# kento/TEZip

Measured on AMD Instinct MI355X. Metric: frames/sec (predict+delta-encode), 512x512 seq, higher is better.
Workload: dtype f32; 1 GPU; 512x512x3 synthetic turbulence stack, 80 frames per GPU (ONE 80-frame sequence), SWP 20-frame windows, warm_up 0, lossy rel 1e-3, entropy remap on; PredNet (3,48,96,192) glorot seed 123

## Files before the change

### tezip_amd/build.py

```python
import os
import subprocess
import sys
from concurrent.futures import ThreadPoolExecutor

HERE = os.path.dirname(os.path.abspath(__file__))
CSRC = os.path.join(HERE, "csrc")
SOURCES = ["tz_api.hip", "tz_codec.hip", "tz_prednet.hip"]
HEADERS = ["tz_internal.h", "tz_math.hip.h", "tz_conv_kernels.hip.h", "tz_wino_kernels.hip.h", "tz_wino_geometry.inc.h", "tz_wino_transform.inc.h",
           "tz_wino_output.inc.h", "tz_wino_epilogue.inc.h", os.path.join("..", "..", "include", "tezip_hip.h")]
LIB = os.path.join(CSRC, "libtezip_hip.so")
HIPCC = os.environ.get("HIPCC", "/opt/rocm/bin/hipcc")
FLAGS = (["-D" + d for d in os.environ.get("TEZIP_DEFINES", "").split()] if os.environ.get("TEZIP_DEFINES") else []) + ["--offload-arch=gfx950", "-O3", "-std=c++17", "-fPIC", "-ffp-contract=off",
         "-fhip-fp32-correctly-rounded-divide-sqrt", "-fno-fast-math", "-Wall", "-Wno-unused-function"]


STAMP = os.path.join(CSRC, ".build_flags")


def _flags_changed():
    try:
        return open(STAMP).read() != " ".join(FLAGS)
    except OSError:
        return True


def _stale(target, deps):
    if not os.path.exists(target):
        return True
    t = os.path.getmtime(target)
    return any(os.path.getmtime(d) > t for d in deps)


def build(force=False, verbose=False):
    hdrs = [os.path.join(CSRC, h) for h in HEADERS]
    force = force or _flags_changed()
    objs, jobs = [], []
    for s in SOURCES:
        src = os.path.join(CSRC, s)
        obj = os.path.join(CSRC, s.replace(".hip", ".o"))
        objs.append(obj)
        if force or _stale(obj, [src] + hdrs):
            jobs.append([HIPCC] + FLAGS + ["-c", src, "-o", obj])

    def run(cmd):
        if verbose:
            print(" ".join(cmd), flush=True)
        r = subprocess.run(cmd, capture_output=True, text=True)
        if r.returncode != 0:
            raise RuntimeError("hipcc failed:\n%s\n%s" % (" ".join(cmd), r.stderr[-8000:]))
        return r.stderr

    if jobs:
        with ThreadPoolExecutor(max_workers=len(jobs)) as ex:
            for err in ex.map(run, jobs):
                if verbose and err.strip():
                    print(err)
    if jobs or force or _stale(LIB, objs):
        run([HIPCC, "--offload-arch=gfx950", "-shared", "-fPIC", "-pthread", "-o", LIB] + objs)
        with open(STAMP, "w") as f:
            f.write(" ".join(FLAGS))
    return LIB


if __name__ == "__main__":
    print(build(force="--force" in sys.argv, verbose=True))
```

### tezip_amd/csrc/tz_prednet.hip

```cpp
#include <algorithm>
#include <atomic>
#include <cmath>

#include "tz_conv_kernels.hip.h"
#include "tz_wino_kernels.hip.h"

struct Seg {
    int row_off, C;
    int up;
    int half = 0;
    int row(int c) const { return half && c >= half ? 4 + c - half : c; }
};
struct PackedConv {
    float* d_W = nullptr;
    float* d_Wimg = nullptr;
    float* d_Wblk = nullptr;
    float* d_Wblk0 = nullptr;
    bool pos_finite = false;
    std::vector<float> h_W0;
    float* d_Wlat = nullptr;
    float* d_Wwino = nullptr;
    float* d_Wwino2 = nullptr;
    const float* d_zero = nullptr;
    float* d_bias = nullptr;
    int nslots = 0, ncols = 0, NT = 1, ncb = 1;
    int wino_finite = 0;
    bool wino_all_finite = false;
    std::vector<Seg> segs;
};

enum { UNI_G0 = 0, UNI_C0 = 1, UNI_AHAT0 = 2 };
enum { UNI_USE_WINO_INIT = 1, UNI_USE_WINO_CELL = 2, UNI_USE_TILES = 4, UNI_USE_ALL = 7 };

struct tz_model {
    int L = 0;
    int stack[TZ_MAX_LEVELS] = {0}, rstack[TZ_MAX_LEVELS] = {0};
    std::vector<std::vector<float>> w;
    int Hp = 0, Wp = 0, maxB = 0;
    int cap = 0;
    bool prepared = false;
    float *R0[TZ_MAX_LEVELS] = {0}, *C0[TZ_MAX_LEVELS] = {0}, *Ahat0[TZ_MAX_LEVELS] = {0}, *G0[TZ_MAX_LEVELS] = {0};
    float *G0f[TZ_MAX_LEVELS] = {0}, *C0f[TZ_MAX_LEVELS] = {0};
    int ring[3][TZ_MAX_LEVELS] = {{0}};
    int tring[3][TZ_MAX_LEVELS] = {{0}};
    const float* uni[3][TZ_MAX_LEVELS] = {{0}};
    int uniform_mask = 0;
    int dead[TZ_MAX_LEVELS] = {0}, dead_gate[TZ_MAX_LEVELS] = {0}, dead_a[TZ_MAX_LEVELS] = {0};
    bool dead0 = false;
    bool dead0_hold = false;
    bool deadf[TZ_MAX_LEVELS] = {false};
    bool deadhalf[TZ_MAX_LEVELS] = {false};
    bool e0_dirty = false;
    float *E[TZ_MAX_LEVELS] = {0}, *R1[TZ_MAX_LEVELS] = {0};
    float* P[TZ_MAX_LEVELS] = {0};
    int Pcap[TZ_MAX_LEVELS] = {0};
    std::vector<signed char> epart_choice;
    PackedConv a_conv[TZ_MAX_LEVELS], gate_t1[TZ_MAX_LEVELS], ahat0_t1;
    PackedConv gate_nf[TZ_MAX_LEVELS];
    float* d_zero = nullptr;
    int e0s = 0;
    int* d_idx = nullptr;
    std::vector<void*> allocs;
    const float* a_k(int l) const { return w[2 * l].data(); }
    const float* a_b(int l) const { return w[2 * l + 1].data(); }
    const float* ahat_k(int l) const { return w[2 * (L - 1) + 2 * l].data(); }
    const float* ahat_b(int l) const { return w[2 * (L - 1) + 2 * l + 1].data(); }
    int gate_base(int g) const {
        static const int pos[4] = {2, 1, 0, 3};
        return 2 * (L - 1) + 2 * L + pos[g] * 2 * L;
    }
    const float* g_k(int g, int l) const { return w[gate_base(g) + 2 * l].data(); }
    const float* g_b(int g, int l) const { return w[gate_base(g) + 2 * l + 1].data(); }
    int gate_cin(int l) const { return rstack[l] + 2 * stack[l] + (l < L - 1 ? rstack[l + 1] : 0); }
};

static int dmalloc(tz_ctx* ctx, tz_model* m, void** p, size_t bytes) {
    if (bytes == 0) bytes = 16;
    hipError_t e = hipMalloc(p, bytes);
    if (e != hipSuccess) return tz_fail(ctx, TZ_ERR_NOMEM, "hipMalloc(%zu) failed: %s", bytes, hipGetErrorString(e));
    m->allocs.push_back(*p);
    return tz_poison(ctx, *p, bytes);
}

struct ColSrc {
    const float* kernel;
    const float* bias;
    int Cin, Cout, ch;
};

static int collapse_set(int a, int d, int out[2]) {
    if (a == 0) {
        if (d == 0) { out[0] = 0; return 1; }
        out[0] = 1; out[1] = 2; return 2;
    }
    if (d == 0) { out[0] = 0; out[1] = 1; return 2; }
    out[0] = 2; return 1;
}

static int pack_conv(tz_ctx* ctx, tz_model* m, const std::vector<Seg>& segs, const std::vector<ColSrc>& cols, int NT,
                     PackedConv* pc) {
    int ncols = (int)cols.size();
    int nslots = 0;
    for (auto& s : segs) nslots += (s.up ? 16 : 9) * ((s.C + 15) / 16);
    std::vector<float> W((size_t)std::max(nslots, 1) * 16 * ncols, 0.0f), B(ncols, 0.0f);
    int slot = 0;
    bool pos_finite = true;
    auto put = [&](const Seg& s, int c0, const int* kys, int nky, const int* kxs, int nkx) {
        for (int kc = 0; kc < 16 && c0 + kc < s.C; ++kc)
            for (int col = 0; col < ncols; ++col) {
                const ColSrc& cs = cols[col];
                if (cs.ch < 0) continue;
                float v = 0.0f;
                bool first = true;
                for (int iy = 0; iy < nky; ++iy)
                    for (int ix = 0; ix < nkx; ++ix) {
                        float w = cs.kernel[((size_t)(kys[iy] * 3 + kxs[ix]) * cs.Cin + s.row_off + c0 + kc) * cs.Cout + cs.ch];
                        v = first ? w : v + w;
                        first = false;
                    }
                W[((size_t)slot * 16 + s.row(c0 + kc) - c0) * ncols + col] = v;
                if (s.half && c0 + kc < s.half && !std::isfinite(v)) pos_finite = false;
            }
        ++slot;
    };
    for (auto& s : segs)
        for (int c0 = 0; c0 < s.C; c0 += 16) {
            if (!s.up) {
                for (int tap = 0; tap < 9; ++tap) {
                    int ky = tap / 3, kx = tap % 3;
                    put(s, c0, &ky, 1, &kx, 1);
                }
            } else {
                for (int tp = 0; tp < 4; ++tp)
                    for (int cls = 0; cls < 4; ++cls) {
                        int kys[2], kxs[2];
// ... 302 lines not shown
    if (epi == EPI_POOL_ERR && !ups) return NT == 4 ? launch_wino_t<4, EPI_POOL_ERR, false>(ctx, a, nbatch) : launch_wino_t<3, EPI_POOL_ERR, false>(ctx, a, nbatch);
    return tz_fail(ctx, TZ_ERR_UNSUPPORTED, "no TZ-PA2 kernel for NT=%d epilogue=%d upsampled=%d", NT, epi, (int)ups);
}

static constexpr long long TZ_PA2_MIN_PIXELS = 256 * 256;
static constexpr size_t kPBytes = (size_t)160 << 20;
static constexpr double kEpartMinIdle = 0.06;
static constexpr int kEpartSteps = 3;
static constexpr int kEpartSamples = 4;
static constexpr float kEpartMinGain = 0.98f;
static int effective_contract(const tz_ctx* ctx) {
    if (ctx->contract) return ctx->contract;
    const tz_model* m = ctx->model;
    return m && (long long)m->Hp * m->Wp >= TZ_PA2_MIN_PIXELS ? 2 : 1;
}

#ifdef TZW_STAMPS
extern "C" int tz_debug_wino_stamps(unsigned long long* out) {
    return hipMemcpyFromSymbol(out, HIP_SYMBOL(tzw_stamps), sizeof(unsigned long long) * 8 * 4096 * 16) == hipSuccess ? 0 : -3;
}
#endif
extern "C" int tz_set_contract(tz_ctx* ctx, int contract) {
    if (!ctx) return TZ_ERR_INVALID;
    if (contract < 0 || contract > 2)
        return tz_fail(ctx, TZ_ERR_INVALID, "tz_set_contract: %d is not 0 (by frame size), 1 (TZ-PA1) or 2 (TZ-PA2)", contract);
    ctx->contract = contract;
    return TZ_OK;
}
extern "C" int tz_get_contract(tz_ctx* ctx) { return ctx ? effective_contract(ctx) : TZ_ERR_INVALID; }

extern "C" int tz_set_conv_impl(tz_ctx* ctx, int lds_dma) {
    if (!ctx) return TZ_ERR_INVALID;
    if (lds_dma < 0 || lds_dma > 5 || (lds_dma >> 1) > 2)
        return tz_fail(ctx, TZ_ERR_INVALID, "tz_set_conv_impl: %d is not 0 / 1 (+ 2 = never k_convlat, + 4 = k_convlat wherever eligible)", lds_dma);
    ctx->conv_impl = (lds_dma & 1) ? 1 : 0;
    const int lat = lds_dma >> 1;
    ctx->lat_mode = lat == 1 ? 0 : (lat == 2 ? 2 : 1);
    return TZ_OK;
}

struct LatPlan {
    bool use, wide;
    int blocks;
};
static LatPlan lat_plan(const tz_ctx* ctx, int NT, int epi, bool ups, bool fullk, const ConvArgs& a, int nbatch) {
    LatPlan lp = {false, false, 0};
    if (!(a.Wlat && a.nsrc > 0 && fullk && ctx->conv_impl && ctx->lat_mode && (NT == 3 || NT == 4) &&
          (epi == EPI_POOL_ERR || (epi == EPI_LSTM && NT == 4))))
        return lp;
    const int ts_ = (epi != EPI_POOL_ERR && ups) ? 8 : 4;
    const long long wg16 = (long long)a.ncb * a.tiles_x * a.tiles_y * nbatch;
    const long long rows_ = (a.H + ts_ - 1) / ts_ * (ts_ == 8 ? 4 : 1);
    const long long wglat1 = (long long)a.ncb * ((a.W + ts_ - 1) / ts_) * rows_ * nbatch;
    const long long wglat2 = (long long)a.ncb * ((a.W + 2 * ts_ - 1) / (2 * ts_)) * rows_ * nbatch;
    static const long long wide_min = getenv("TEZIP_LAT_WIDE_MIN") ? atoll(getenv("TEZIP_LAT_WIDE_MIN")) : 2560;
    lp.wide = wglat1 > wide_min;
    int slots = 0;
    for (int s = 0; s < a.nsrc; ++s) slots += a.src[s].cpt * (a.src[s].up ? 4 : 9);
    const double t16 = slots * 1.08 * (double)((wg16 + 255) / 256);
    const double per_slot = lp.wide ? 0.134 * (double)((wglat2 + 255) / 256) : std::max(0.105, 0.078 * (double)((wglat1 + 255) / 256));
    const double tlat = slots * per_slot * (ts_ == 8 ? 1.1 : 1.0) + 2.5;
    lp.use = wg16 <= 768 && (ctx->lat_mode == 2 || tlat < 0.9 * t16);
    lp.blocks = (int)(lp.wide ? wglat2 : wglat1);
    return lp;
}

static int launch_conv(tz_ctx* ctx, int NT, int epi, const ConvArgs& a, int nbatch, int wino_dead = 0, const float* wino3 = nullptr,
                       const float* wino3q = nullptr) {
    tz_prof_scope ps(ctx, TZP_CONV);
    bool ups = false, fullk = true;
    for (int s = 0; s < a.nsrc; ++s) {
        ups = ups || a.src[s].up;
        fullk = fullk && (a.src[s].C % 16) == 0;
        const long long hs = a.src[s].up ? a.H >> 1 : a.H, ws = a.src[s].up ? a.W >> 1 : a.W;
        fullk = fullk && hs * ws * a.src[s].pstride * 4 < (1LL << 32);
    }
    ps.sub = TZP_CONV_GEN;
    if (epi == EPI_RELU && a.nsrc == 1 && !ups && a.src[0].C == 3 && a.Cout == 3 && ctx->conv_impl) {
        ps.sub = TZP_CONV_SMALL;
        hipLaunchKernelGGL((k_conv_small<3, 3>), dim3(a.tiles_x * a.tiles_y * nbatch), dim3(256), 0, ctx->stream, a);
        TZ_HIP(ctx, hipGetLastError());
        return TZ_OK;
    }
    if (a.Wblk && a.nsrc > 0 && !a.src[0].up && a.src[0].pstride == 8 && ctx->conv_impl) {
        const int blocks = a.ncb * a.tiles_x * a.tiles_y * nbatch;
#define TZ_CASE16B(nt, e, u)                                                                                    \
    if (NT == nt && epi == e && ups == u) {                                                                     \
        ps.sub = TZP_CONV16B;                                                                                   \
        if (a.Wblk0) hipLaunchKernelGGL((k_conv16b<nt, e, u, true>), dim3(blocks), dim3(NTHR), 0, ctx->stream, a); \
        else hipLaunchKernelGGL((k_conv16b<nt, e, u>), dim3(blocks), dim3(NTHR), 0, ctx->stream, a);            \
        TZ_HIP(ctx, hipGetLastError());                                                                         \
        return TZ_OK;                                                                                           \
    }
        TZ_CASE16B(1, EPI_LSTM_PACKED, true) TZ_CASE16B(1, EPI_LSTM_PACKED, false)
        TZ_CASE16B(1, EPI_POOL_ERR, false) TZ_CASE16B(3, EPI_POOL_ERR, false) TZ_CASE16B(4, EPI_POOL_ERR, false)
#undef TZ_CASE16B
    }
    if (a.Wwino && effective_contract(ctx) == 2 && fullk && (epi == EPI_LSTM || epi == EPI_POOL_ERR || epi == EPI_RAW)) {
        ps.sub = TZP_WINO;
        return launch_wino(ctx, NT, epi, ups, a, nbatch, false, wino_dead, wino3, wino3q);
    }
    {
        const LatPlan lp = lat_plan(ctx, NT, epi, ups, fullk, a, nbatch);
        if (!lp.use) goto no_lat;
        const bool wide = lp.wide;
        const int blocks = lp.blocks;
        ps.sub = TZP_CONVLAT;
#define TZ_LAT(e, u)                                                                                          \
    do {                                                                                                      \
        if (wide) hipLaunchKernelGGL((k_convlat<e, u, 2>), dim3(blocks), dim3(256), 0, ctx->stream, a);       \
        else hipLaunchKernelGGL((k_convlat<e, u, 1>), dim3(blocks), dim3(256), 0, ctx->stream, a);            \
    } while (0)
        if (epi == EPI_LSTM && ups) TZ_LAT(EPI_LSTM, true);
        else if (epi == EPI_LSTM) TZ_LAT(EPI_LSTM, false);
        else TZ_LAT(EPI_POOL_ERR, false);
#undef TZ_LAT
        TZ_HIP(ctx, hipGetLastError());
        return TZ_OK;
    }
no_lat:
    if (a.Wimg && a.nsrc > 0 && fullk && ctx->conv_impl) {
#define TZ_CASE16(nt, e, u)                          \
    if (NT == nt && epi == e && ups == u) {          \
        ps.sub = TZP_CONV16;                         \
        launch_conv16_t<nt, e, u>(ctx, a, nbatch);   \
        TZ_HIP(ctx, hipGetLastError());              \
        return TZ_OK;                                \
    }
        TZ_CASE16(4, EPI_LSTM, false) TZ_CASE16(4, EPI_LSTM, true)
        TZ_CASE16(3, EPI_POOL_ERR, false) TZ_CASE16(4, EPI_POOL_ERR, false)
#undef TZ_CASE16
    }
#define TZ_CASE(nt, e, u)                                                   \
    if (NT == nt && epi == e && ups == u) {                                 \
        if (fullk) launch_conv_t<nt, e, u, true>(ctx, a, nbatch);           \
        else launch_conv_t<nt, e, u, false>(ctx, a, nbatch);                \
        TZ_HIP(ctx, hipGetLastError());                                     \
        return TZ_OK;                                                       \
    }
    TZ_CASE(1, EPI_RAW, false) TZ_CASE(4, EPI_RAW, false)
    TZ_CASE(1, EPI_RELU, false) TZ_CASE(3, EPI_RELU, false) TZ_CASE(4, EPI_RELU, false)
    TZ_CASE(4, EPI_LSTM, false) TZ_CASE(4, EPI_LSTM, true)
    TZ_CASE(1, EPI_LSTM_PACKED, false) TZ_CASE(1, EPI_LSTM_PACKED, true)
    TZ_CASE(1, EPI_POOL_ERR, false) TZ_CASE(3, EPI_POOL_ERR, false) TZ_CASE(4, EPI_POOL_ERR, false)
#undef TZ_CASE
    return tz_fail(ctx, TZ_ERR_UNSUPPORTED, "no conv kernel for NT=%d epilogue=%d upsampled=%d", NT, epi, (int)ups);
}

static void fill_srcs(ConvArgs& a, const PackedConv& pc, const float* const* ptrs, const long long* nstrides,
                      int pstride0 = 0) {
    a.nsrc = (int)pc.segs.size();
    for (int s = 0; s < a.nsrc; ++s) {
        a.src[s].p = ptrs[s];
        a.src[s].nstride = nstrides[s];
        a.src[s].C = pc.segs[s].half ? 8 : pc.segs[s].C;
        a.src[s].pstride = s == 0 && pstride0 ? pstride0 : pc.segs[s].C;
        a.src[s].up = pc.segs[s].up;
        a.src[s].cpt = (pc.segs[s].C + 15) / 16;
    }
    a.Wp = pc.d_W;
    a.Wimg = pc.d_Wimg;
    a.Wblk = pc.d_Wblk;
    a.Wblk0 = pc.d_Wblk0;
    a.Wlat = pc.d_Wlat;
    a.Wwino = pc.d_Wwino;
    a.zero = pc.d_zero;
// ... 164 lines not shown
        static const char* const names[2] = {"gates", "A"};
        for (int k = 0; k < 2; ++k) {
            if (!pcs[k] || !pcs[k]->d_Wwino) continue;
            *out[k] = pcs[k]->wino_finite >= d ? d : 0;
            if (log)
                fprintf(stderr, "[tezip] dead source, level %d %s: %d of %d leading positive-half blocks dead, %d skipped: %d of %d same-resolution stages%s\n",
                        l, names[k], d, m->stack[l] / 16, *out[k], 4 * *out[k], 2 * m->stack[l] / 4,
                        !on ? " (TEZIP_DEADSRC=0)" : (*out[k] < d ? " (a weight of those stages is not finite)" : ""));
        }
    }
    for (int l = 0; l < L; ++l) {
        const bool whole = l == 0 ? half0 : (m->stack[l] % 16 == 0 && m->stack[l] / 16 <= 64);
        const unsigned long long blocks = l == 0 ? 1ull : (m->stack[l] / 16 >= 64 ? ~0ull : (1ull << (m->stack[l] / 16)) - 1);
        m->deadhalf[l] = onh && whole && !(h_live[l] & blocks);
        if (logh)
            fprintf(stderr, "[tezip] dead half, level %d: Ahat0 +-0 over the whole plane: %s%s\n", l, m->deadhalf[l] ? "yes" : "no",
                    m->deadhalf[l] ? " (its writers store the live half alone)" : !onh ? " (TEZIP_DEADHALF=0)" : "");
    }
    if (half0 && (on0 || log0)) {
        const bool zero = !(h_live[0] & 1);
        m->dead0 = zero;
        PackedConv* pcs[2] = {L > 1 ? &m->a_conv[0] : nullptr, &m->gate_t1[0]};
        static const char* const names[2] = {"A", "gates"};
        for (int k = 0; k < 2; ++k) {
            if (!pcs[k]) continue;
            const bool form = pcs[k]->d_Wblk && !pcs[k]->h_W0.empty() && (k == 0 || pcs[k]->NT == 1), finite = pcs[k]->pos_finite;
            if (on0 && zero && form && finite) TZ_TRY(pack_block0_dead(ctx, m, pcs[k]));
            if (log0)
                fprintf(stderr, "[tezip] dead level 0, %s: positive half of E_0 +0 everywhere: %s, its k-step left out: %s%s\n", names[k],
                        zero ? "yes" : "no", pcs[k]->d_Wblk0 ? "yes" : "no",
                        pcs[k]->d_Wblk0 ? " (9 of 18 k-steps in block 0 of k_conv16b)"
                        : !zero         ? ""
                        : !on0          ? " (TEZIP_DEAD0=0)"
                        : !form         ? " (no k_conv16b form)"
                                        : " (a weight of those rows is not finite)");
        }
    }
    return TZ_OK;
}

static int measure_deadf(tz_ctx* ctx, tz_model* m) {
    const int L = m->L;
    const char* env = getenv("TEZIP_DEADF");
    const bool on = !env || atoi(env) != 0;
    const bool log = getenv("TEZIP_DEADF_LOG") && atoi(getenv("TEZIP_DEADF_LOG"));
    unsigned long long h_live[TZ_MAX_LEVELS] = {0};
    for (int l = 0; l < TZ_MAX_LEVELS; ++l) m->deadf[l] = false;
    if (!on && !log) return TZ_OK;
    {
        unsigned long long* d_live = nullptr;
        TZ_TRY(dmalloc(ctx, m, (void**)&d_live, sizeof(h_live)));
        TZ_HIP(ctx, hipMemsetAsync(d_live, 0, sizeof(h_live), ctx->stream));
        for (int l = 1; l < L; ++l) {
            const long long nwords = (long long)(m->Hp >> l) * (m->Wp >> l) * m->rstack[l];
            hipLaunchKernelGGL(k_live_blocks, dim3((unsigned)std::min<long long>((nwords + 255) / 256, 4096)), dim3(256), 0, ctx->stream,
                               (const unsigned*)m->C0[l], nwords, 1, 1, d_live + l, 0xffffffffu);
            TZ_HIP(ctx, hipGetLastError());
        }
        TZ_HIP(ctx, hipMemcpyAsync(h_live, d_live, sizeof(h_live), hipMemcpyDeviceToHost, ctx->stream));
        TZ_HIP(ctx, hipStreamSynchronize(ctx->stream));
    }
    for (int l = 1; l < L; ++l) {
        const bool zero = !(h_live[l] & 1);
        const bool form = m->gate_t1[l].d_Wwino && m->gate_t1[l].NT == 4;
        const bool finite = form && m->gate_t1[l].wino_all_finite;
        m->deadf[l] = on && zero && form && finite;
        if (m->deadf[l]) {
            std::vector<ColSrc> cols, cols3;
            int NT;
            TZ_TRY(gate_cols(ctx, m, l, &cols, &NT));
            for (size_t c = 0; c < cols.size(); ++c)
                if ((c % 64) / 16 != 1) cols3.push_back(cols[c]);
            TZ_TRY(pack_wino(ctx, m, m->gate_t1[l].segs, cols3, 3, &m->gate_nf[l]));
            m->deadf[l] = m->gate_nf[l].d_Wwino != nullptr;
        }
        if (log)
            fprintf(stderr, "[tezip] dead forget gate, level %d: C0 +0 everywhere: %s, forget-gate columns left out: %s%s\n", l, zero ? "yes" : "no",
                    m->deadf[l] ? "yes" : "no",
                    m->deadf[l] ? " (3 of 4 column tiles in every k_wino gate launch, fused or split)"
                    : !zero     ? ""
                    : !on       ? " (TEZIP_DEADF=0)"
                    : !form     ? " (no k_wino form)"
                                : " (a weight of the convolution is not finite)");
    }
    return TZ_OK;
}

static int choose_wino_forms(tz_ctx* ctx, tz_model* m) {
    const char* env = getenv("TEZIP_WINO2Q");
    const bool on = !env || atoi(env) != 0;
    const bool log = getenv("TEZIP_WINO2Q_LOG") && atoi(getenv("TEZIP_WINO2Q_LOG"));
    for (int l = 1; l < m->L; ++l)
        for (int k = 0; k < 2; ++k) {
            if (k == 1 && l == m->L - 1) continue;
            PackedConv& pc = k == 0 ? (m->deadf[l] ? m->gate_nf[l] : m->gate_t1[l]) : m->a_conv[l];
            pc.d_Wwino2 = nullptr;
            if (!pc.d_Wwino) continue;
            const int s_full = (2 * m->stack[l]) / 4, s_up = k == 0 && l < m->L - 1 ? m->rstack[l + 1] / 4 : 0;
            const int dead = k == 0 ? m->dead_gate[l] : m->dead_a[l];
            const int s_same = dead > 0 && 16 * (dead + 1) <= 2 * m->stack[l] ? s_full - 4 * dead : s_full;
            const bool three = k == 0 ? m->deadf[l] : pc.NT == 3;
            const bool walk = wino2q_walk(s_same, s_up, s_full - s_same, s_full + s_up);
            if (on && three && walk) {
                const long long nquads = (long long)(k == 0 ? m->gate_t1[l].ncb : pc.ncb) * (s_full + s_up);
                TZ_TRY(dmalloc(ctx, m, (void**)&pc.d_Wwino2, (size_t)nquads * 3072 * 4));
                hipLaunchKernelGGL(k_dense_stages, dim3((unsigned)std::min<long long>((nquads * 3072 + 255) / 256, 4096)), dim3(256), 0, ctx->stream,
                                   pc.d_Wwino, pc.d_Wwino2, nquads);
                TZ_HIP(ctx, hipGetLastError());
            }
            if (log)
                fprintf(stderr, "[tezip] k_wino stage, level %d %s: %d + %d stages, %s: %s\n", l, k == 0 ? "gates" : "A", s_same, s_up,
                        three ? "three column tiles" : "four column tiles",
                        pc.d_Wwino2 ? "two-quad (k_wino2)"
                        : !three    ? "one-quad"
                        : !on       ? "one-quad (TEZIP_WINO2Q=0)"
                                    : "one-quad (stages not a multiple of 6)");
        }
    TZ_HIP(ctx, hipStreamSynchronize(ctx->stream));
    return TZ_OK;
}

extern "C" int tz_model_prepare(tz_ctx* ctx, int Hp, int Wp, int max_batch) {
    tz_roctx_range roctx_("tz_model_prepare");
    if (!ctx) return TZ_ERR_INVALID;
    tz_model* m = ctx->model;
    if (!m) return tz_fail(ctx, TZ_ERR_STATE, "tz_model_prepare before tz_model_load");
    const int L = m->L;
    if (Hp <= 0 || Wp <= 0 || max_batch < 1) return tz_fail(ctx, TZ_ERR_INVALID, "bad prepare arguments");
    if ((Hp % (1 << (L - 1))) || (Wp % (1 << (L - 1))) || (Hp % 8) || (Wp % 8))
        return tz_fail(ctx, TZ_ERR_INVALID,
                       "Image size is out of scope for this model: padded size %dx%d must divide by 8 and 2^(levels-1)", Hp, Wp);
    long long limit_px = -1;
    for (int l = 0; l < L; ++l) {
        const long long widest = std::max<long long>(4LL * m->rstack[l], std::max<long long>(2LL * m->stack[l], 8));
        const long long lim = (((1LL << 30) - 1) / widest) << (2 * l);
        if (limit_px < 0 || lim < limit_px) limit_px = lim;
    }
    for (int l = 0; l < L; ++l) {
        const long long npx = (long long)(Hp >> l) * (Wp >> l);
        const long long widest = std::max<long long>(4LL * m->rstack[l], std::max<long long>(2LL * m->stack[l], 8));
        if (npx * widest >= (1LL << 30))
            return tz_fail(ctx, TZ_ERR_UNSUPPORTED,
                           "frame of %dx%d pixels: level %d holds %lld floats per frame, the kernels address a frame's plane with 32-bit "
                           "offsets (< 2^30 floats); this model accepts frames up to about %lld pixels",
                           Hp, Wp, l, npx * widest, limit_px);
    }
    if (m->prepared && m->Hp == Hp && m->Wp == Wp && m->maxB >= max_batch) {
        m->cap = max_batch;
        return TZ_OK;
    }
    {
        std::vector<std::vector<float>> w = std::move(m->w);
        int st[TZ_MAX_LEVELS], rs[TZ_MAX_LEVELS];
        for (int l = 0; l < L; ++l) { st[l] = m->stack[l]; rs[l] = m->rstack[l]; }
        tz_model_free(ctx);
        m = new tz_model();
        ctx->model = m;
        m->L = L;
        for (int l = 0; l < L; ++l) { m->stack[l] = st[l]; m->rstack[l] = rs[l]; }
        m->w = std::move(w);
    }
    m->Hp = Hp;
    m->Wp = Wp;
    m->maxB = max_batch;
    m->cap = max_batch;
    m->epart_choice.assign((size_t)max_batch + 1, (signed char)-1);
// ... 26 lines not shown
        std::vector<ColSrc> cols;
        int NT;
        TZ_TRY(gate_cols(ctx, m, l, &cols, &NT));
        std::vector<Seg> segs;
        if (l < L - 1) segs.push_back(Seg{m->rstack[l] + 2 * m->stack[l], m->rstack[l + 1], 1});
        PackedConv pc;
        TZ_TRY(pack_conv(ctx, m, segs, cols, NT, &pc));
        ConvArgs a;
        memset(&a, 0, sizeof(a));
        const float* ptrs[2] = {l < L - 1 ? m->R0[l + 1] : nullptr, nullptr};
        long long ns[2] = {0, 0};
        fill_srcs(a, pc, ptrs, ns);
        set_geom(a, hl(l), wl(l));
        a.Cout = m->rstack[l];
        a.R = m->rstack[l];
        a.out0 = m->R0[l];
        a.out1 = m->C0[l];
        TZ_TRY(launch_conv(ctx, NT, NT == 4 ? EPI_LSTM : EPI_LSTM_PACKED, a, 1));
    }
    for (int l = 0; l < L; ++l) {
        int Cout = m->stack[l], NT = plain_nt(Cout);
        PackedConv pc;
        TZ_TRY(pack_conv(ctx, m, {Seg{0, m->rstack[l], 0}}, plain_cols(m->ahat_k(l), m->ahat_b(l), m->rstack[l], Cout), NT, &pc));
        if (l == 0) m->ahat0_t1 = pc;
        ConvArgs a;
        memset(&a, 0, sizeof(a));
        const float* ptrs[2] = {m->R0[l], nullptr};
        long long ns[2] = {0, 0};
        fill_srcs(a, pc, ptrs, ns);
        set_geom(a, hl(l), wl(l));
        a.Cout = Cout;
        a.out0 = m->Ahat0[l];
        a.clip1 = l == 0;
        TZ_TRY(launch_conv(ctx, NT, EPI_RELU, a, 1));
    }
    for (int l = 0; l < L; ++l) {
        std::vector<ColSrc> cols;
        int NT;
        TZ_TRY(gate_cols(ctx, m, l, &cols, &NT));
        PackedConv pg;
        TZ_TRY(pack_conv(ctx, m, {Seg{0, m->rstack[l], 0}}, cols, NT, &pg));
        size_t npx = (size_t)hl(l) * wl(l);
        TZ_TRY(dmalloc(ctx, m, (void**)&m->G0[l], npx * pg.ncols * 4));
        ConvArgs a;
        memset(&a, 0, sizeof(a));
        const float* ptrs[2] = {m->R0[l], nullptr};
        long long ns[2] = {0, 0};
        fill_srcs(a, pg, ptrs, ns);
        set_geom(a, hl(l), wl(l));
        a.out0 = m->G0[l];
        TZ_TRY(launch_conv(ctx, NT, EPI_RAW, a, 1));
        const int half = l == 0 && m->e0s == 8 ? m->stack[0] : 0;
        std::vector<Seg> segs = {Seg{m->rstack[l], 2 * m->stack[l], 0, half}};
        if (l < L - 1) segs.push_back(Seg{m->rstack[l] + 2 * m->stack[l], m->rstack[l + 1], 1});
        TZ_TRY(pack_conv(ctx, m, segs, cols, NT, &m->gate_t1[l]));
        if (l >= 1) TZ_TRY(pack_wino(ctx, m, segs, cols, NT, &m->gate_t1[l]));
        {
            const int tx = (wl(l) + 15) / 16, ty = (hl(l) + 15) / 16, ncb = pg.ncols / (16 * NT);
            const bool parity = l < L - 1;
            const size_t nf = (size_t)tx * ty * ncb * 8 * 2 * NT * 256;
            TZ_TRY(dmalloc(ctx, m, (void**)&m->G0f[l], nf * 4));
            if (parity) hipLaunchKernelGGL(k_to_fragments<MAP_PARITY>, dim3(1024), dim3(256), 0, ctx->stream, m->G0[l], hl(l), wl(l), tx, ty, pg.ncols, ncb, NT, m->G0f[l]);
            else hipLaunchKernelGGL(k_to_fragments<MAP_LINEAR>, dim3(1024), dim3(256), 0, ctx->stream, m->G0[l], hl(l), wl(l), tx, ty, pg.ncols, ncb, NT, m->G0f[l]);
            TZ_HIP(ctx, hipGetLastError());
            if (NT == 4) {
                const size_t nc = (size_t)tx * ty * ncb * 8 * 2 * 256;
                TZ_TRY(dmalloc(ctx, m, (void**)&m->C0f[l], nc * 4));
                if (parity) hipLaunchKernelGGL(k_to_fragments<MAP_PARITY>, dim3(1024), dim3(256), 0, ctx->stream, m->C0[l], hl(l), wl(l), tx, ty, m->rstack[l], ncb, 1, m->C0f[l]);
                else hipLaunchKernelGGL(k_to_fragments<MAP_LINEAR>, dim3(1024), dim3(256), 0, ctx->stream, m->C0[l], hl(l), wl(l), tx, ty, m->rstack[l], ncb, 1, m->C0f[l]);
                TZ_HIP(ctx, hipGetLastError());
            }
        }
    }
    for (int l = 0; l < L - 1; ++l) {
        int Cout = m->stack[l + 1], NT = plain_nt(Cout);
        const int half = l == 0 && m->e0s == 8 ? m->stack[0] : 0;
        TZ_TRY(pack_conv(ctx, m, {Seg{0, 2 * m->stack[l], 0, half}}, plain_cols(m->a_k(l), m->a_b(l), 2 * m->stack[l], Cout), NT,
                         &m->a_conv[l]));
        if (l >= 1) TZ_TRY(pack_wino(ctx, m, {Seg{0, 2 * m->stack[l], 0}}, plain_cols(m->a_k(l), m->a_b(l), 2 * m->stack[l], Cout), NT, &m->a_conv[l]));
    }
    TZ_TRY(measure_uniform(ctx, m));
    TZ_TRY(measure_dead(ctx, m));
    TZ_TRY(measure_deadf(ctx, m));
    TZ_TRY(choose_wino_forms(ctx, m));
    m->prepared = true;
    return TZ_OK;
}

int tz_model_dims(tz_ctx* ctx, int* Hp, int* Wp, int* max_batch) {
    tz_model* m = ctx->model;
    if (!m || !m->prepared) return tz_fail(ctx, TZ_ERR_STATE, "model not prepared");
    *Hp = m->Hp;
    *Wp = m->Wp;
    *max_batch = m->cap;
    return TZ_OK;
}

int tz_model_c0_dev(tz_ctx* ctx, const float** c0) {
    tz_model* m = ctx->model;
    if (!m || !m->prepared) return tz_fail(ctx, TZ_ERR_STATE, "model not prepared");
    *c0 = m->Ahat0[0];
    return TZ_OK;
}

int tz_model_predict_batch(tz_ctx* ctx, int n, const int* h_in_is_key, const int* h_in_idx, const int* h_out_idx,
                           const uint8_t* d_frames_u8, int H, int W, const float* d_in_stack, float* d_out_stack) {
    tz_model* m = ctx->model;
    if (!m || !m->prepared) return tz_fail(ctx, TZ_ERR_STATE, "model not prepared");
    if (n < 1 || n > m->maxB) return tz_fail(ctx, TZ_ERR_INVALID, "batch %d outside 1..%d", n, m->maxB);
    std::vector<int> idx(3 * (size_t)m->maxB, 0);
    for (int i = 0; i < n; ++i) {
        idx[i] = h_in_is_key[i];
        idx[m->maxB + i] = h_in_idx[i];
        idx[2 * m->maxB + i] = h_out_idx[i];
    }
    TZ_TRY(tz_upload(ctx, m->d_idx, idx.data(), sizeof(int) * idx.size()));
    return tz_model_predict_batch_dev(ctx, n, m->d_idx, m->maxB, d_frames_u8, H, W, d_in_stack, d_out_stack, 0);
}

static bool epart_levels(tz_ctx* ctx, tz_model* m, int n, bool* lv, double* idle) {
    const int L = m->L;
    for (int l = 0; l < TZ_MAX_LEVELS; ++l) lv[l] = false;
    *idle = 0.0;
    if (!(effective_contract(ctx) == 2 && ctx->conv_impl && ctx->stream2 && !ctx->split_rollout)) return false;
    auto hl = [&](int l) { return m->Hp >> l; };
    auto wl = [&](int l) { return m->Wp >> l; };
    double busy = 0.0, span = 0.0;
    for (int l = 1; l < L; ++l) {
        const long long tiles = (long long)((hl(l) + 15) / 16) * ((wl(l) + 15) / 16) * n;
        const int s_e = (2 * m->stack[l]) / 4, s_u = l < L - 1 ? m->rstack[l + 1] / 4 : 0;
        const long long it[2] = {m->gate_t1[l].d_Wwino ? tiles * m->gate_t1[l].ncb : 0,
                                 l < L - 1 && m->a_conv[l].d_Wwino ? tiles * m->a_conv[l].ncb : 0};
        const int st[2] = {s_e - 4 * m->dead_gate[l] + s_u, s_e - 4 * m->dead_a[l]};
        const double len[2] = {m->deadf[l] ? 0.75 : 1.0, 1.0};
        for (int k = 0; k < 2; ++k) {
            if (!it[k]) continue;
            busy += (double)it[k] / ctx->num_cus * st[k] * len[k];
            span += (double)((it[k] + ctx->num_cus - 1) / ctx->num_cus) * st[k] * len[k];
        }
    }
    if (span > 0.0) *idle = 1.0 - busy / span;
    bool any = false;
    for (int l = 1; l < L - 1; ++l) {
        lv[l] = m->P[l] && n <= m->Pcap[l] && m->gate_t1[l].d_Wwino && m->gate_t1[l].NT == 4 && m->gate_t1[l].segs.size() == 2 &&
                (m->rstack[l + 1] % 16) == 0 && (2 * m->stack[l]) % 16 == 0;
        any = any || lv[l];
    }
    return any;
}

static int predict_batch_impl(tz_ctx* ctx, int n, const int* d_idx, int stride, const uint8_t* d_frames_u8, int H, int W,
                              const float* d_in_stack, float* d_out_stack, int slot0, const int* d_next_slot, bool skip_err0,
                              bool* fused_next, bool err0_keys_only, bool use_epart);

static int epart_measure(tz_ctx* ctx, int n, const int* d_idx, int stride, const uint8_t* d_frames_u8, int H, int W,
                         const float* d_in_stack, float* d_out_stack, int slot0, const int* d_next_slot, int* choice) {
    if (!ctx->ev_cal[0]) {
        TZ_HIP(ctx, hipEventCreate(&ctx->ev_cal[0]));
        hipError_t e = hipEventCreate(&ctx->ev_cal[1]);
        if (e != hipSuccess) {
            (void)hipEventDestroy(ctx->ev_cal[0]);
            ctx->ev_cal[0] = nullptr;
            ctx->ev_cal[1] = nullptr;
            TZ_HIP(ctx, e);
        }
    }
// ... 373 lines not shown
```

Measured before the change: 3430 frames/s.

## Add vector-ALU level-0 gate kernel that skips dead forget gate

Adds a dedicated k_l0_gates kernel for the level-0 LSTM gate convolution (3 channels, upsampled R1 source). It uses packed f32x2 FMAs, a tiled LDS layout for the frame and the upsampled R1 planes, and double-buffered weight and activation requests. At prepare time it checks that the level-0 cell state C0 is all zeros and the weights are finite, then drops the forget-gate columns, computing 9 of 12. This is meant to replace k_conv16b for this launch and avoid matrix-core padding waste on a tiny channel count. The cost is a specialised code path that depends on the measured zero state.

```diff
diff --git a/tezip_amd/build.py b/tezip_amd/build.py
--- a/tezip_amd/build.py
+++ b/tezip_amd/build.py
@@ -7,7 +7,7 @@
 CSRC = os.path.join(HERE, "csrc")
 SOURCES = ["tz_api.hip", "tz_codec.hip", "tz_prednet.hip"]
 HEADERS = ["tz_internal.h", "tz_math.hip.h", "tz_conv_kernels.hip.h", "tz_wino_kernels.hip.h", "tz_wino_geometry.inc.h", "tz_wino_transform.inc.h",
-           "tz_wino_output.inc.h", "tz_wino_epilogue.inc.h", os.path.join("..", "..", "include", "tezip_hip.h")]
+           "tz_wino_output.inc.h", "tz_wino_epilogue.inc.h", "tz_l0_kernels.hip.h", os.path.join("..", "..", "include", "tezip_hip.h")]
 LIB = os.path.join(CSRC, "libtezip_hip.so")
 HIPCC = os.environ.get("HIPCC", "/opt/rocm/bin/hipcc")
 FLAGS = (["-D" + d for d in os.environ.get("TEZIP_DEFINES", "").split()] if os.environ.get("TEZIP_DEFINES") else []) + ["--offload-arch=gfx950", "-O3", "-std=c++17", "-fPIC", "-ffp-contract=off",
diff --git a/tezip_amd/csrc/tz_l0_kernels.hip.h b/tezip_amd/csrc/tz_l0_kernels.hip.h
--- /dev/null
+++ b/tezip_amd/csrc/tz_l0_kernels.hip.h
@@ -0,0 +1,210 @@
+#pragma once
+#include "tz_conv_kernels.hip.h"
+
+typedef float f32x2 __attribute__((ext_vector_type(2)));
+
+namespace tzl0 {
+
+typedef const __attribute__((address_space(4))) f32x2* cpair;
+__device__ __forceinline__ cpair as_const(const float* p) { return (cpair)(unsigned long long)p; }
+
+__device__ __forceinline__ f32x2 fma2(float x, f32x2 w, f32x2 acc) { return __builtin_elementwise_fma((f32x2){x, x}, w, acc); }
+
+__device__ __forceinline__ f32x2 zero2() {
+    f32x2 z = {0.0f, 0.0f};
+    asm volatile("" : "+v"(z));
+    return z;
+}
+
+__device__ __forceinline__ float add_zero(float x) {
+    float r;
+    asm("v_add_f32 %0, 0, %1" : "=v"(r) : "v"(x));
+    return r;
+}
+
+}
+
+namespace tzl0 {
+static constexpr int GT = 32;
+static constexpr int EW = GT + 2;
+static constexpr int RW = GT / 2 + 2;
+static constexpr int RPIX = RW * RW;
+static constexpr int R_ITEMS = (RPIX * 4 + 255) / 256;
+template <int NP>
+__device__ __forceinline__ constexpr int pair_col(int p) { return NP == 6 ? 2 * p : (p < 2 ? 2 * p : 2 * p + 2); }
+template <int NP>
+__device__ __forceinline__ float col_of(const f32x2 (&acc)[NP], int col) {
+    return NP == 6 || col < 4 ? acc[col >> 1][col & 1] : acc[(col - 2) >> 1][col & 1];
+}
+}
+
+template <bool DEAD0, int NP>
+__global__ __launch_bounds__(256, DEAD0 && NP == 5 ? 4 : 3) void k_l0_gates(const ConvArgs a, const float* wg) {
+    using namespace tzl0;
+    constexpr int NQ = DEAD0 ? 1 : 2;
+    constexpr int LDSQ = NQ * EW * EW > 16 * RPIX / 4 ? NQ * EW * EW : 16 * RPIX / 4;
+    __shared__ f32x4 smem[LDSQ];
+    float* const planes = (float*)smem;
+    const int tid = threadIdx.x, lane = tid & 63, cls = __builtin_amdgcn_readfirstlane(tid >> 6);
+    const int pa = cls >> 1, pb = cls & 1;
+    const int tx32 = (a.W + GT - 1) / GT, ty32 = (a.H + GT - 1) / GT;
+    const int tile = blockIdx.x % (tx32 * ty32), n = blockIdx.x / (tx32 * ty32);
+    const int ty0 = (tile / tx32) * GT, tx0 = (tile % tx32) * GT;
+    const int H2 = a.H >> 1, W2 = a.W >> 1;
+    const int nub = a.src[1].cpt;
+
+    const float* r1 = a.src[1].p + (long long)n * a.src[1].nstride;
+    const int rps = a.src[1].pstride;
+    f32x4 pre[R_ITEMS];
+    auto fetch_r1 = [&](int b) {
+#pragma unroll
+        for (int k = 0; k < R_ITEMS; ++k) {
+            const int i = tid + 256 * k, px = i >> 2, q = i & 3;
+            const int Y = px / RW, X = px - Y * RW;
+            const int ly = (ty0 >> 1) - 1 + Y, lx = (tx0 >> 1) - 1 + X;
+            pre[k] = (f32x4){0.0f, 0.0f, 0.0f, 0.0f};
+            if (px < RPIX && ly >= 0 && ly < H2 && lx >= 0 && lx < W2) pre[k] = *(const f32x4*)(r1 + ((long long)ly * W2 + lx) * rps + b * 16 + 4 * q);
+        }
+    };
+    auto store_r1 = [&]() {
+#pragma unroll
+        for (int k = 0; k < R_ITEMS; ++k) {
+            const int i = tid + 256 * k, px = i >> 2, q = i & 3;
+            if (px < RPIX) {
+#pragma unroll
+                for (int c = 0; c < 4; ++c) planes[(4 * q + c) * RPIX + px] = pre[k][c];
+            }
+        }
+    };
+    if (nub > 0) fetch_r1(0);
+    {
+        const float* base = a.src[0].p + (long long)n * a.src[0].nstride;
+        for (int i = tid; i < NQ * EW * EW; i += 256) {
+            const int q = DEAD0 ? 1 : i / (EW * EW), slot = DEAD0 ? i : i - q * (EW * EW);
+            const int y = slot / EW, x = slot - y * EW;
+            const int yy = ty0 - 1 + y, xx = tx0 - 1 + x;
+            f32x4 v = {0.0f, 0.0f, 0.0f, 0.0f};
+            if (yy >= 0 && yy < a.H && xx >= 0 && xx < a.W) v = *(const f32x4*)(base + ((long long)yy * a.W + xx) * 8 + 4 * q);
+            smem[i] = v;
+        }
+    }
+    const int by = lane >> 2, bxg = lane & 3;
+    const int y = ty0 + 2 * by + pa, x0 = tx0 + 8 * bxg + pb;
+    f32x2 acc[4][NP];
+#pragma unroll
+    for (int k = 0; k < 4; ++k) {
+        const int x = x0 + 2 * k;
+        const long long pix = (y < a.H && x < a.W) ? (long long)y * a.W + x : 0;
+#pragma unroll
+        for (int p = 0; p < NP; ++p) acc[k][p] = *(const f32x2*)(a.init + pix * a.ncols + pair_col<NP>(p));
+    }
+    const f32x2 z = zero2();
+    __syncthreads();
+#pragma unroll
+    for (int dy = 0; dy < 3; ++dy) {
+        f32x4 xr[NQ][9];
+#pragma unroll
+        for (int q = 0; q < NQ; ++q)
+#pragma unroll
+            for (int j = 0; j < 9; ++j) xr[q][j] = smem[q * (EW * EW) + (2 * by + pa + dy) * EW + 8 * bxg + pb + j];
+#pragma unroll
+        for (int dx = 0; dx < 3; ++dx) {
+            const int tap = dy * 3 + dx;
+#pragma unroll
+            for (int q = 0; q < NQ; ++q) {
+#pragma unroll
+                for (int ch = 0; ch < 3; ++ch) {
+                    const float* wrow = a.Wp + (tap * 16 + 4 * (DEAD0 ? 1 : q) + ch) * a.ncols;
+                    f32x2 w[NP];
+#pragma unroll
+                    for (int p = 0; p < NP; ++p) w[p] = as_const(wrow + pair_col<NP>(p))[0];
+#pragma unroll
+                    for (int k = 0; k < 4; ++k)
+#pragma unroll
+                        for (int p = 0; p < NP; ++p) acc[k][p] = fma2(xr[q][2 * k + dx][ch], w[p], acc[k][p]);
+                }
+#pragma unroll
+                for (int k = 0; k < 4; ++k)
+#pragma unroll
+                    for (int p = 0; p < NP; ++p) acc[k][p] = acc[k][p] + z;
+            }
+        }
+    }
+    const float* xbase = planes + (by + pa) * RW + 4 * bxg + pb;
+#pragma unroll 1
+    for (int b = 0; b < nub; ++b) {
+        __syncthreads();
+        store_r1();
+        __syncthreads();
+        if (b + 1 < nub) fetch_r1(b + 1);
+        const float* wblk = wg + (long long)(cls * nub + b) * (64 * 12);
+        auto request = [&](int s, f32x2 (&w)[2][6], float (&xv)[2][4]) {
+            const int tp = s >> 3, c0 = 2 * (s & 7);
+            const cpair wrow = as_const(wblk + s * 24);
+            const float* xp = xbase + c0 * RPIX + (tp >> 1) * RW + (tp & 1);
+#pragma unroll
+            for (int c = 0; c < 2; ++c) {
+#pragma unroll
+                for (int p = 0; p < 6; ++p) w[c][p] = wrow[6 * c + p];
+#pragma unroll
+                for (int k = 0; k < 4; ++k) xv[c][k] = xp[c * RPIX + k];
+            }
+        };
+        auto landed = [&]() {
+            __builtin_amdgcn_s_waitcnt(0xc07f);
+            __builtin_amdgcn_sched_barrier(0);
+        };
+        auto compute = [&](const f32x2 (&w)[2][6], const float (&xv)[2][4]) {
+#pragma unroll
+            for (int c = 0; c < 2; ++c)
+#pragma unroll
+                for (int k = 0; k < 4; ++k)
+#pragma unroll
+                    for (int p = 0; p < NP; ++p) acc[k][p] = fma2(xv[c][k], w[c][pair_col<NP>(p) >> 1], acc[k][p]);
+            __builtin_amdgcn_sched_barrier(0);
+        };
+        f32x2 wa[2][6], wb[2][6];
+        float xa[2][4], xb[2][4];
+        request(0, wa, xa);
+        landed();
+#pragma unroll 1
+        for (int s = 0; s < 32; s += 2) {
+            request(s + 1, wb, xb);
+            compute(wa, xa);
+            landed();
+            request(s + 2, wa, xa);
+            compute(wb, xb);
+            landed();
+        }
+    }
+    constexpr int R = 3;
+    float* o0 = a.out0 + (long long)n * a.out0_nstride;
+    float* o1 = a.out1 ? a.out1 + (long long)n * a.out1_nstride : nullptr;
+#pragma unroll
+    for (int k = 0; k < 4; ++k) {
+        const int x = x0 + 2 * k;
+        const bool ok = y < a.H && x < a.W;
+        const long long pix = ok ? (long long)y * a.W + x : 0;
+#pragma unroll
+        for (int c = 0; c < R; ++c) {
+            const float gi = tz_hard_sigmoid(col_of<NP>(acc[k], c));
+            const float gg = tz_tanh(col_of<NP>(acc[k], 2 * R + c));
+            const float go = tz_hard_sigmoid(col_of<NP>(acc[k], 3 * R + c));
+            const float t2 = gi * gg;
+            float cc;
+            if (NP == 6) {
+                const float gf = tz_hard_sigmoid(col_of<NP>(acc[k], R + c));
+                const float cp = a.aux ? a.aux[pix * R + c] : 0.0f;
+                const float t1 = gf * cp;
+                cc = t1 + t2;
+            } else {
+                cc = add_zero(t2);
+            }
+            const float rr = go * tz_tanh(cc);
+            if (ok) {
+                o0[pix * R + c] = rr;
+                if (o1) o1[pix * R + c] = cc;
+            }
+        }
+    }
+}
diff --git a/tezip_amd/csrc/tz_prednet.hip b/tezip_amd/csrc/tz_prednet.hip
--- a/tezip_amd/csrc/tz_prednet.hip
+++ b/tezip_amd/csrc/tz_prednet.hip
@@ -4,6 +4,7 @@
 
 #include "tz_conv_kernels.hip.h"
 #include "tz_wino_kernels.hip.h"
+#include "tz_l0_kernels.hip.h"
 
 struct Seg {
     int row_off, C;
@@ -51,6 +52,8 @@
     bool deadf[TZ_MAX_LEVELS] = {false};
     bool deadhalf[TZ_MAX_LEVELS] = {false};
     bool e0_dirty = false;
+    bool l0valu_g = false, deadf0 = false;
+    float* l0_wg = nullptr;
     float *E[TZ_MAX_LEVELS] = {0}, *R1[TZ_MAX_LEVELS] = {0};
     float* P[TZ_MAX_LEVELS] = {0};
     int Pcap[TZ_MAX_LEVELS] = {0};
@@ -519,6 +522,15 @@
         TZ_HIP(ctx, hipGetLastError());
         return TZ_OK;
     }
+    if (const tz_model* m = ctx->model; m && ctx->conv_impl && a.nsrc > 0 && a.src[0].pstride == 8) {
+        if (m->l0valu_g && a.Wblk0 && epi == EPI_LSTM_PACKED && ups && a.nsrc == 2 && a.init && a.Wp == m->gate_t1[0].d_W) {
+            ps.sub = TZP_CONV16B;
+            const int blocks = ((a.W + tzl0::GT - 1) / tzl0::GT) * ((a.H + tzl0::GT - 1) / tzl0::GT) * nbatch;
+            hipLaunchKernelGGL((k_l0_gates<true, 5>), dim3(blocks), dim3(256), 0, ctx->stream, a, m->l0_wg);
+            TZ_HIP(ctx, hipGetLastError());
+            return TZ_OK;
+        }
+    }
     if (a.Wblk && a.nsrc > 0 && !a.src[0].up && a.src[0].pstride == 8 && ctx->conv_impl) {
         const int blocks = a.ncb * a.tiles_x * a.tiles_y * nbatch;
 #define TZ_CASE16B(nt, e, u)                                                                                    \
@@ -849,6 +861,59 @@
                     : !on       ? " (TEZIP_DEADF=0)"
                     : !form     ? " (no k_wino form)"
                                 : " (a weight of the convolution is not finite)");
+    }
+    return TZ_OK;
+}
+
+static int choose_l0_forms(tz_ctx* ctx, tz_model* m) {
+    const char* env = getenv("TEZIP_L0VALU");
+    const bool on = !env || atoi(env) != 0;
+    const bool log = getenv("TEZIP_L0VALU_LOG") && atoi(getenv("TEZIP_L0VALU_LOG"));
+    m->l0valu_g = m->deadf0 = false;
+    m->l0_wg = nullptr;
+    const bool shape = m->L > 1 && m->stack[0] == 3 && m->rstack[0] == 3 && m->e0s == 8 && m->rstack[1] % 16 == 0;
+    const PackedConv& pg = m->gate_t1[0];
+    const bool form_g = shape && pg.d_Wblk && pg.NT == 1 && pg.ncols == 16 && pg.segs.size() == 2;
+    bool zero = false, finite = false;
+    if (on && form_g) {
+        unsigned long long h_live = 0, *d_live = nullptr;
+        TZ_TRY(dmalloc(ctx, m, (void**)&d_live, sizeof(h_live)));
+        TZ_HIP(ctx, hipMemsetAsync(d_live, 0, sizeof(h_live), ctx->stream));
+        const long long nwords = (long long)m->Hp * m->Wp * m->rstack[0];
+        hipLaunchKernelGGL(k_live_blocks, dim3((unsigned)std::min<long long>((nwords + 255) / 256, 4096)), dim3(256), 0, ctx->stream,
+                           (const unsigned*)m->C0[0], nwords, 1, 1, d_live, 0xffffffffu);
+        TZ_HIP(ctx, hipGetLastError());
+        TZ_HIP(ctx, hipMemcpyAsync(&h_live, d_live, sizeof(h_live), hipMemcpyDeviceToHost, ctx->stream));
+        TZ_HIP(ctx, hipStreamSynchronize(ctx->stream));
+        zero = !(h_live & 1);
+        std::vector<float> W((size_t)pg.nslots * 16 * pg.ncols);
+        TZ_HIP(ctx, hipMemcpy(W.data(), pg.d_W, W.size() * 4, hipMemcpyDeviceToHost));
+        finite = true;
+        for (float v : W) finite = finite && std::isfinite(v);
+        const int nub = pg.segs[1].C / 16;
+        std::vector<float> G((size_t)4 * nub * 64 * 12 + 24, 0.0f);
+        for (int cls = 0; cls < 4; ++cls)
+            for (int b = 0; b < nub; ++b)
+                for (int tp = 0; tp < 4; ++tp)
+                    for (int ch = 0; ch < 16; ++ch)
+                        for (int c = 0; c < 12; ++c)
+                            G[((((size_t)cls * nub + b) * 4 + tp) * 16 + ch) * 12 + c] = W[((size_t)(9 + 16 * b + 4 * tp + cls) * 16 + ch) * pg.ncols + c];
+        TZ_TRY(dmalloc(ctx, m, (void**)&m->l0_wg, G.size() * 4));
+        TZ_HIP(ctx, hipMemcpy(m->l0_wg, G.data(), G.size() * 4, hipMemcpyHostToDevice));
+        const char* envf = getenv("TEZIP_DEADF");
+        m->deadf0 = zero && finite && (!envf || atoi(envf) != 0);
+        m->l0valu_g = m->deadf0 && pg.d_Wblk0 != nullptr;
+    }
+    if (log) {
+        fprintf(stderr, "[tezip] level 0 A: k_conv16b (its vector-ALU form was not faster: EXPERIMENTS.md)\n");
+        fprintf(stderr, "[tezip] level 0 gates: %s%s\n", m->l0valu_g ? "k_l0_gates (vector ALU)" : "k_conv16b",
+                m->l0valu_g   ? ", forget-gate columns left out: yes (9 of 12 gate columns)"
+                : !on         ? " (TEZIP_L0VALU=0)"
+                : !form_g     ? " (not the reference shape)"
+                : !pg.d_Wblk0 ? " (the positive half of E_0 is walked: k_conv16b is the faster form)"
+                : !zero       ? " (the forget gate is needed: k_conv16b is the faster form)"
+                : !finite     ? " (a weight of the convolution is not finite: the forget gate is needed)"
+                              : " (TEZIP_DEADF=0: the forget gate is kept)");
     }
     return TZ_OK;
 }
@@ -1041,6 +1106,7 @@
     TZ_TRY(measure_uniform(ctx, m));
     TZ_TRY(measure_dead(ctx, m));
     TZ_TRY(measure_deadf(ctx, m));
+    TZ_TRY(choose_l0_forms(ctx, m));
     TZ_TRY(choose_wino_forms(ctx, m));
     m->prepared = true;
     return TZ_OK;
```

Result: faster. 3482 frames/s, median of 6 (+1.5%).
